# zfw1226/active_tracking_rl

Measured on AMD Instinct MI355X. Metric: env steps/sec, Track2D-BlockPartialPZR-v0 @4096 envs, 1/2/4/8 GPU, higher is better.
Workload: dtype u8 map bits / f64 reward -> f32 obs+reward; policy fp32

## Files before the change

### active_tracking_rl_amd/build.py

```python
import os
import re
import subprocess
import sys
from concurrent.futures import ThreadPoolExecutor

HERE = os.path.dirname(os.path.abspath(__file__))
CSRC = os.path.join(HERE, "csrc")
OBJ = os.path.join(CSRC, "_obj")
LIB = os.path.join(HERE, "libtrack2d_hip.so")
SOURCES = ["track2d_hip.hip", "stem_hip.hip", "policy_hip.hip", "lstm_hip.hip", "heads_hip.hip", "gemm_tn_hip.hip",
           "actor_step_hip.hip", "pair_gemm_hip.hip", "bptt_hip.hip", "driver_hip.hip", "gate_cell_hip.hip", "episode_stats_hip.hip",
           "gru_hip.hip", "np_mode.cpp", "lt_gemm.cpp"]
HEADERS = ["t2d_device.h", os.path.join("..", "..", "include", "track2d.h"),
           os.path.join("..", "..", "include", "atr_policy.h"), "atr_sample.h", "atr_cell.h",
           os.path.join("..", "..", "include", "track2d_np.h"), os.path.join("..", "..", "include", "atr_eval.h"),
           os.path.join("..", "..", "include", "atr_stats.h"), os.path.join("..", "..", "include", "atr_gru.h"),
           os.path.join("..", "..", "include", "atr_gru_step.h"), os.path.join("..", "..", "include", "atr_gru_sums.h")]
HIPCC = os.environ.get("HIPCC", "/opt/rocm/bin/hipcc")
CFLAGS = ["--offload-arch=gfx950", "-O3", "-std=c++17", "-ffp-contract=off", "-fPIC", "-Wno-unused-result"]
LDFLAGS = ["--offload-arch=gfx950", "-fPIC", "-shared", "-ldl"]
NO_SCRATCH = {"track2d_hip.hip": "k_gru_step"}
NO_SCRATCH_LEARNER = {"gru_hip.hip": "k_gru_bptt"}
REMARKS = "-Rpass-analysis=kernel-resource-usage"


def _newest_header():
    return max(os.path.getmtime(os.path.join(CSRC, h)) for h in HEADERS)


def _obj(src):
    return os.path.join(OBJ, os.path.splitext(src)[0] + ".o")


def _stale(src, hdr_time):
    o = _obj(src)
    return not os.path.exists(o) or os.path.getmtime(o) < max(os.path.getmtime(os.path.join(CSRC, src)), hdr_time)


def needs_build():
    if not os.path.exists(LIB):
        return True
    t = os.path.getmtime(LIB)
    return any(os.path.getmtime(os.path.join(CSRC, f)) > t for f in SOURCES + HEADERS)


# ... 4 lines not shown
        if m:
            name = m.group(1)
            seen += part in name
            continue
        m = re.search(r"remark:\s+ScratchSize \[bytes/lane\]: (\d+)", line)
        if m and name is not None and part in name and int(m.group(1)) != 0:
            bad.append((name, int(m.group(1))))
    if not seen:
        raise RuntimeError("no resource remark names a %s kernel: the scratch check found nothing to check" % part)
    return bad


def build(force=False, verbose=False):
    if not force and not needs_build():
        return LIB
    os.makedirs(OBJ, exist_ok=True)
    hdr_time = _newest_header()
    todo = [s for s in SOURCES if force or _stale(s, hdr_time)]

    def compile_one(src):
        cmd = [HIPCC] + CFLAGS + ["-c", os.path.join(CSRC, src), "-o", _obj(src)]
        if verbose:
            print(" ".join(cmd), flush=True)
        part = NO_SCRATCH.get(src) or NO_SCRATCH_LEARNER.get(src)
        if part is None:
            subprocess.check_call(cmd)
            return
        r = subprocess.run(cmd + [REMARKS], stderr=subprocess.PIPE, text=True)
        if r.returncode != 0:
            sys.stderr.write(r.stderr)
            raise subprocess.CalledProcessError(r.returncode, cmd)
        sys.stderr.write("".join(l + "\n" for l in r.stderr.splitlines() if "warning:" in l))
        bad = scratch_users(r.stderr, part)
        if bad:
            os.remove(_obj(src))
            raise RuntimeError("%s: scratch memory in %s" % (src, ", ".join("%s (%d bytes per lane)" % b for b in bad)))
    with ThreadPoolExecutor(max_workers=min(len(todo), os.cpu_count() or 4) or 1) as pool:
        list(pool.map(compile_one, todo))
    cmd = [HIPCC] + LDFLAGS + ["-o", LIB] + [_obj(s) for s in SOURCES]
    if verbose:
        print(" ".join(cmd), flush=True)
    subprocess.check_call(cmd)
    return LIB


if __name__ == "__main__":
    print(build(force="--force" in sys.argv, verbose=True))
# ... 1 lines not shown
```

### active_tracking_rl_amd/csrc/heads_hip.hip

```cpp
#include <hip/hip_runtime.h>
#include <stdint.h>

#include "../../include/atr_policy.h"

namespace atr {

constexpr int kHeadsMaxA = 8;
constexpr int kHeadsBlock = 256;

__device__ __forceinline__ float4 h_ld4(const float *p) { return *reinterpret_cast<const float4 *>(p); }
__device__ __forceinline__ float dot4(const float4 &a, const float4 &b) { return fmaf(a.x, b.x, fmaf(a.y, b.y, fmaf(a.z, b.z, a.w * b.w))); }
__device__ __forceinline__ float row_sum(float v, int L)
{
    v += __builtin_bit_cast(float, __builtin_amdgcn_update_dpp(0, __builtin_bit_cast(int, v), 0xB1 , 0xf, 0xf, true));
    v += __builtin_bit_cast(float, __builtin_amdgcn_update_dpp(0, __builtin_bit_cast(int, v), 0x4E , 0xf, 0xf, true));
    v += __builtin_bit_cast(float, __builtin_amdgcn_update_dpp(0, __builtin_bit_cast(int, v), 0x124 , 0xf, 0xf, true));
    v += __builtin_bit_cast(float, __builtin_amdgcn_update_dpp(0, __builtin_bit_cast(int, v), 0x128 , 0xf, 0xf, true));
    if (L > 16) v += __shfl_xor(v, 16, 64);
    if (L > 32) v += __shfl_xor(v, 32, 64);
    return v;
}

__global__ __launch_bounds__(kHeadsBlock) void k_heads_values(const float *__restrict__ h, const float *__restrict__ wc,
                                                              const float *__restrict__ bc, float *__restrict__ values,
                                                              long long rows, int R, int vstride, int voff,
                                                              const float *__restrict__ h1, const float *__restrict__ wc1,
                                                              const float *__restrict__ bc1, int voff1)
{
    const int half = h1 ? (int)(gridDim.x >> 1) : (int)gridDim.x;
    const bool second = h1 && (int)blockIdx.x >= half;
    if (second) { h = h1; wc = wc1; bc = bc1; voff = voff1; }
    const int bid = second ? (int)blockIdx.x - half : (int)blockIdx.x;
    const int L = R >> 2;
    const long long total = rows * L;
// ... 46 lines not shown
    const float4 wc = h_ld4(a.wc + j);
    const float4 wx = a.waux ? h_ld4(a.waux + j) : make_float4(0.f, 0.f, 0.f, 0.f);
    const long long rstride = (long long)nblk * slots;
    long long row = (long long)bid * slots + slot;
    float4 hv_n = make_float4(0.f, 0.f, 0.f, 0.f);
    float v_n = 0.f, ret_n = 0.f, gae_n = 0.f, raux_n = 0.f;
    int act_n_ = 0;
    auto fetch = [&](long long r) {
        if (r < a.rows) {
            hv_n = h_ld4(a.h + r * a.R + j);
            const long long s_ = r * a.stride + a.off;
            v_n = a.val[s_]; ret_n = a.ret[s_]; gae_n = a.gae[s_];
            const unsigned an_ = (unsigned)(a.act_n > 0x7fffffffLL ? 0x7fffffffLL : a.act_n), at_ = (unsigned)r / an_;
            act_n_ = (int)a.actions[(long long)at_ * a.act_tstride + (long long)((unsigned)r - at_ * an_)];
            if (a.r_aux) raux_n = a.r_aux[r * a.aux_stride + a.aux_off];
        }
    };
    fetch(row);
    for (; row < a.rows; row += rstride) {
        const float4 hv = hv_n;
        const float v = v_n, ret = ret_n, gae = gae_n, raux = raux_n;
        const int act = act_n_;
        fetch(row + rstride);
        float z[NAx];
#pragma unroll
        for (int i = 0; i < NAx; i++) z[i] = i < A ? row_sum(dot4(hv, wa[i]), L) + a.ba[i] : -INFINITY;
        const float pred = a.waux ? row_sum(dot4(hv, wx), L) + a.baux[0] : 0.f;
        float mx = z[0];
#pragma unroll
        for (int i = 1; i < NAx; i++) mx = fmaxf(mx, z[i]);
        float p[NAx], se = 0.f;
#pragma unroll
        for (int i = 0; i < NAx; i++) { p[i] = i < A ? expf(z[i] - mx) : 0.f; se += p[i]; }
        const float lse = mx + logf(se);
        float ent = 0.f, logp_a = 0.f;
#pragma unroll
        for (int i = 0; i < NAx; i++) {
            if (i < A) {
                p[i] = p[i] / se;
                const float lp = z[i] - lse;
                ent -= lp * p[i];
                if (i == act) logp_a = lp;
            }
        }
        const float dlogp = -a.scale * gae, dent = -a.scale * a.w_ent;
        const float dv = a.scale * 0.5f * (v - ret);
        float dpred = 0.f, aux_abs = 0.f;
        if (a.r_aux) {
            const float diff = pred - raux;
            aux_abs = fabsf(diff);
            dpred = a.scale_aux * (diff > 0.f ? 1.f : (diff < 0.f ? -1.f : 0.f));
        }
        float dz[NAx];
#pragma unroll
        for (int i = 0; i < NAx; i++)
            dz[i] = i < A ? dlogp * ((i == act ? 1.f : 0.f) - p[i]) - dent * p[i] * ((z[i] - lse) + ent) : 0.f;
        float4 dh = make_float4(dv * wc.x + dpred * wx.x, dv * wc.y + dpred * wx.y, dv * wc.z + dpred * wx.z, dv * wc.w + dpred * wx.w);
#pragma unroll
        for (int i = 0; i < NAx; i++)
            if (i < A) {
                dh.x = fmaf(dz[i], wa[i].x, dh.x); dh.y = fmaf(dz[i], wa[i].y, dh.y);
                dh.z = fmaf(dz[i], wa[i].z, dh.z); dh.w = fmaf(dz[i], wa[i].w, dh.w);
                gwa[i].x = fmaf(dz[i], hv.x, gwa[i].x); gwa[i].y = fmaf(dz[i], hv.y, gwa[i].y);
                gwa[i].z = fmaf(dz[i], hv.z, gwa[i].z); gwa[i].w = fmaf(dz[i], hv.w, gwa[i].w);
                gba[i] += dz[i];
            }
        {
            float *dp = a.dh + row * a.R + j;
            __builtin_nontemporal_store(dh.x, dp); __builtin_nontemporal_store(dh.y, dp + 1);
            __builtin_nontemporal_store(dh.z, dp + 2); __builtin_nontemporal_store(dh.w, dp + 3);
        }
        gwc.x = fmaf(dv, hv.x, gwc.x); gwc.y = fmaf(dv, hv.y, gwc.y); gwc.z = fmaf(dv, hv.z, gwc.z); gwc.w = fmaf(dv, hv.w, gwc.w);
        gwx.x = fmaf(dpred, hv.x, gwx.x); gwx.y = fmaf(dpred, hv.y, gwx.y); gwx.z = fmaf(dpred, hv.z, gwx.z); gwx.w = fmaf(dpred, hv.w, gwx.w);
        gbc += dv; gbx += dpred;
        s_pol += -logp_a * gae - a.w_ent * ent;
        s_val += 0.5f * (ret - v) * (ret - v);
        s_ent += ent;
        s_aux += aux_abs;
    }
    __shared__ float4 wred[kHeadsBlock];
    const int rec = (A + 2) * a.R + (A + 2) + 4;
    float *out = a.partial + (size_t)bid * rec;
#pragma unroll
    for (int q = 0; q < NAx + 2; q++) {
        if (q < A + 2) {
            float4 g = gwx;
            if (q < NAx && q < A) g = gwa[q < NAx ? q : 0];
            else if (q == A) g = gwc;
            __syncthreads();
            wred[threadIdx.x] = g;
            __syncthreads();
            if (slot == 0) {
                float4 acc = wred[threadIdx.x];
                for (int sl = 1; sl < slots; sl++) {
                    const float4 t = wred[sl * L + (int)threadIdx.x];
                    acc.x += t.x; acc.y += t.y; acc.z += t.z; acc.w += t.w;
                }
                *reinterpret_cast<float4 *>(out + q * a.R + j) = acc;
            }
        }
    }
    __syncthreads();
    if (j == 0) {
#pragma unroll
        for (int i = 0; i < NAx; i++) red[slot][i] = gba[i];
        red[slot][kHeadsMaxA] = gbc; red[slot][kHeadsMaxA + 1] = gbx;
        red[slot][kHeadsMaxA + 2] = s_pol; red[slot][kHeadsMaxA + 3] = s_val;
        red[slot][kHeadsMaxA + 4] = s_ent; red[slot][kHeadsMaxA + 5] = s_aux;
    }
    __syncthreads();
    if (threadIdx.x < (unsigned)(A + 2 + 4)) {
        const int q = (int)threadIdx.x;
        const int src = q < A ? q : kHeadsMaxA + (q - A);
        float acc = 0.f;
        for (int sl = 0; sl < slots; sl++) acc += red[sl][src];
        out[(A + 2) * a.R + q] = acc;
    }
}

struct HeadsReduce {
    const float *partial[2];
    float *out[2];
    float *stats_out[2];
    float scale[2], scale_aux[2];
    int nrec[2];
    float stats_scale;
    int rec, nb, fold;
};

__global__ __launch_bounds__(1024) void k_heads_reduce(const HeadsReduce f)
{
    __shared__ float red[64][17];
    __shared__ float tail[16];
    const int pi = (int)blockIdx.x >= f.nb ? 1 : 0, b = (int)blockIdx.x - pi * f.nb;
    const float *__restrict__ partial = f.partial[pi];
    float *__restrict__ out = f.out[pi];
    const int nrec = f.nrec[pi], rec = f.rec;
    const int jl = (int)(threadIdx.x & 15u), slice = (int)(threadIdx.x >> 4);
    const int j = b * 16 + jl;
    float acc = 0.f;
// ... 86 lines not shown
    for (int i = 0; i < 2; i++) {
        const atr_heads_loss_args &p = players[i < count ? i : 0];
        if (heads_fill(g.p[i], p) != 0) return -1;
        if (i >= count) g.p[i].grid = 0;
        f.partial[i] = p.workspace; f.out[i] = p.grads_and_sums; f.stats_out[i] = p.stats_out; f.scale[i] = p.scale;
        f.scale_aux[i] = p.scale_aux; f.nrec[i] = g.p[i].grid;
    }
    if (count == 2 && (players[0].R != players[1].R || players[0].A != players[1].A)) return -1;
    const int rec = (players[0].A + 2) * players[0].R + (players[0].A + 2) + 4;
    f.stats_scale = stats_scale; f.rec = rec; f.nb = (rec + 15) / 16; f.fold = (rec - 4) / 16 == (rec - 1) / 16 ? 1 : 0;
    hipStream_t st = (hipStream_t)stream;
    if (players[0].A <= 4)
        hipLaunchKernelGGL(k_heads_loss<4>, dim3((unsigned)(g.p[0].grid + g.p[1].grid)), dim3(kHeadsBlock), 0, st, g);
    else
        hipLaunchKernelGGL(k_heads_loss<kHeadsMaxA>, dim3((unsigned)(g.p[0].grid + g.p[1].grid)), dim3(kHeadsBlock), 0, st, g);
    hipLaunchKernelGGL(k_heads_reduce, dim3((unsigned)(f.nb * count)), dim3(1024), 0, st, f);
    if (!f.fold)
        for (int i = 0; i < count; i++)
            hipLaunchKernelGGL(k_heads_finish, dim3(1), dim3(1), 0, st, players[i].grads_and_sums, rec, players[i].scale,
                               players[i].scale_aux, players[i].stats_out, stats_scale);
    return hipGetLastError() == hipSuccess ? 0 : -2;
}

extern "C" int atr_heads_loss(const float *h, const long long *actions, const float *ret, const float *gae,
                              const float *val, int stride, int off, const float *r_aux, int aux_stride, int aux_off,
                              const float *wa, const float *ba, const float *wc, const float *waux, const float *baux,
                              float scale, float scale_aux, float w_ent, float *dh, float *grads_and_sums,
                              float *workspace, long long rows, int R, int A, void *stream)
{
    atr_heads_loss_args p = {};
    p.h = h; p.actions = actions; p.act_n = rows > 0 ? rows : 1; p.act_tstride = 0; p.ret = ret; p.gae = gae; p.val = val;
    p.stride = stride; p.off = off; p.r_aux = r_aux; p.aux_stride = aux_stride; p.aux_off = aux_off; p.wa = wa; p.ba = ba;
    p.wc = wc; p.waux = waux; p.baux = baux; p.scale = scale; p.scale_aux = scale_aux; p.w_ent = w_ent; p.dh = dh;
    p.grads_and_sums = grads_and_sums; p.workspace = workspace; p.stats_out = nullptr; p.rows = rows; p.R = R; p.A = A;
    return atr_heads_loss_multi(&p, 1, 1.0f, stream);
}
```

### active_tracking_rl_amd/fused.py

```python
import ctypes as C
import json
import os
import re
import sys

import torch

from . import vec_env

_lib = None


class ActStepArgs(C.Structure):
    _fields_ = [("ig", C.c_void_p * 2), ("hg", C.c_void_p * 2), ("bias", C.c_void_p * 2), ("c_prev", C.c_void_p * 2),
                ("h_out", C.c_void_p * 2), ("c_out", C.c_void_p * 2), ("acts", C.c_void_p * 2),
                ("actor_w", C.c_void_p * 2), ("actor_b", C.c_void_p * 2), ("emb", C.c_void_p), ("done_prev", C.c_void_p),
                ("actions_out", C.c_void_p), ("counter", C.c_void_p), ("seed", C.c_ulonglong), ("ordinal", C.c_uint),
                ("A", C.c_int), ("N", C.c_int), ("R", C.c_int), ("hm_out", C.c_void_p * 2), ("hm_ld", C.c_longlong)]


class CoopStepArgs(C.Structure):
    _fields_ = [("y", C.c_void_p * 2), ("fc_w", C.c_void_p * 2), ("fc_b", C.c_void_p * 2), ("w_cat", C.c_void_p * 2),
                ("ldy", C.c_longlong * 2), ("kfc", C.c_int * 2), ("fh", C.c_void_p), ("gates", C.c_void_p),
                ("fh_pstride", C.c_longlong), ("fh_ld", C.c_longlong), ("F", C.c_int), ("workgroups", C.c_int),
# ... 119 lines not shown


ATR_PROTOTYPES = _prototypes()
GRU_PROTOTYPES = {
    "atr_gru_cell_forward": (C.c_int, [C.c_void_p] * 6 + [C.c_longlong, C.c_void_p, C.c_void_p, C.c_void_p, C.c_longlong,
                                       C.c_void_p, C.c_longlong, C.c_int, C.c_int, C.c_int, C.c_void_p]),
    "atr_gru_cell_backward": (C.c_int, [C.c_void_p, C.c_longlong, C.c_void_p, C.c_void_p, C.c_void_p, C.c_void_p, C.c_longlong,
                                        C.c_void_p, C.c_longlong, C.c_void_p, C.c_longlong, C.c_int, C.c_int, C.c_int, C.c_int,
                                        C.c_void_p]),
    "atr_gru_bptt": (C.c_int, [C.c_void_p] * 4 + [C.c_longlong, C.c_void_p, C.c_longlong, C.c_void_p, C.c_void_p, C.c_void_p,
                               C.c_longlong, C.c_void_p, C.c_int, C.c_int, C.c_int, C.c_int, C.c_void_p]),
}
GRU_SUMS_PROTOTYPES = {
    "atr_gru_bptt_act_sums_floats": (C.c_longlong, [C.c_int]),
    "atr_gru_bptt_sums": (C.c_int, GRU_PROTOTYPES["atr_gru_bptt"][1][:12] + [C.c_int, C.c_int, C.c_void_p, C.c_longlong, C.c_void_p,
                                                                            C.c_int, C.c_int, C.c_int, C.c_int, C.c_void_p]),
}
GRU_STEP_PROTOTYPES = {
    "atr_gru_act_env_step": (C.c_int, [C.c_void_p, C.POINTER(ActStepArgs), C.c_void_p, C.c_void_p, C.c_longlong, C.c_void_p,
                                       C.c_int, C.c_void_p, C.c_void_p, C.c_void_p]),
    "atr_gru_eval_act_env_step": (C.c_int, [C.c_void_p, C.POINTER(ActStepArgs), C.c_void_p, C.c_void_p, C.c_longlong, C.c_void_p,
                                            C.c_void_p, C.c_int, C.c_void_p, C.c_void_p, C.c_void_p]),
}
_ERROR_DETAIL = {"atr_act_env_step": "t2d_last_error", "atr_coop_env_step": "t2d_last_error", "atr_linear": "atr_lt_last_error"}
_GRU_STEP_ERROR_DETAIL = {name: "t2d_last_error" for name in GRU_STEP_PROTOTYPES}


def _errcheck(name):
    def check(status, func=None, args=None):
        if status != 0:
            text = _ERROR_DETAIL.get(name) or _GRU_STEP_ERROR_DETAIL.get(name)
            detail = ": " + getattr(lib(), text)().decode() if text else ""
            raise RuntimeError("%s failed (%d)%s" % (name, status, detail))
        return status
    return check


def lib():
    global _lib
    if _lib is None:
        L = vec_env.load_library()
        for name, (restype, argtypes, *value) in (list(ATR_PROTOTYPES.items()) + list(GRU_PROTOTYPES.items())
                                                  + list(GRU_SUMS_PROTOTYPES.items()) + list(GRU_STEP_PROTOTYPES.items())):
            f = getattr(L, name)
            f.restype, f.argtypes = restype, argtypes
            if restype is C.c_int and not value:
                f.errcheck = _errcheck(name)
        _lib = L
    return _lib


def _p(t):
    return C.c_void_p(t.data_ptr())


def _stem_fn(name, x):
    if x.dtype == torch.uint8:
        return getattr(lib(), name + "_u8")
    if x.dtype != torch.float32:
        raise TypeError("stem frames must be float32 or uint8, got %s" % x.dtype)
    return getattr(lib(), name)


def _stream(t):
    return C.c_void_p(torch.cuda.current_stream(t.device).cuda_stream)

# ... 1130 lines not shown
        return hs[0][1][hs[0][5]], hs[1][1][hs[1][5]], stats

    @staticmethod
    def backward(ctx, g0, g1, gstats):
        sv = ctx.saved_tensors
        out = [None]
        for p in range(2):
            if (g0, g1)[p] is None:
                out += [None] * 7
            else:
                out += _head_grads(sv[2 * p], sv[2 * p + 1], *ctx.dims[p])
        return tuple(out)


def heads_loss_pair(hs, actors, critics, auxes, cfg):
    t = []
    for p in range(2):
        aux = auxes[p]
        t += [hs[p], actors[p].weight, actors[p].bias, critics[p].weight, critics[p].bias,
              aux.weight if aux is not None else None, aux.bias if aux is not None else None]
    return _HeadsLossPair.apply(cfg, *t)


class _HeadsLoss(torch.autograd.Function):

    @staticmethod
    def forward(ctx, h, wa, ba, wc, bc, waux, baux, actions, ret, gae, val, off, r_aux, aux_off, scale, scale_aux, w_ent,
                unit_coeff=False):
        L = lib()
        h = h.contiguous()
        rows, R = h.shape
        A = wa.shape[0]
        stride = _col_stride(ret)
        rec = (A + 2) * R + (A + 2) + 4
        dh = torch.empty_like(h)
        gs = torch.empty(rec + 1, dtype=torch.float32, device=h.device)
        ws = torch.empty(L.atr_heads_workspace_floats(rows, R, A), dtype=torch.float32, device=h.device)
        actions = actions.contiguous()
        aux_stride = _col_stride(r_aux) if r_aux is not None else 0
        L.atr_heads_loss(_p(h), _p(actions), _p(ret), _p(gae), _p(val), stride, off, _pn(r_aux), aux_stride, aux_off,
                         _p(wa), _p(ba), _p(wc), _pn(waux), _pn(baux), float(scale), float(scale_aux), float(w_ent),
                         _p(dh), _p(gs), _p(ws), rows, R, A, _stream(h))
        ctx.save_for_backward(dh, gs)
        ctx.dims = (A, R, waux is not None)
        ctx.unit_coeff = bool(unit_coeff)
        stats = gs[rec - 4:rec]
# ... 270 lines not shown
```

### active_tracking_rl_amd/player_util.py

```python
import torch
import torch.distributed as dist


class Agent(object):
    def __init__(self, model, env, args, state, device):
        self.model = model
        self.env = env
        self.num_agents = len(env.observation_space)
        self.num_envs = getattr(env, "num_envs", 1)
        if 'continuous' in args.network:
            raise NotImplementedError("continuous actions belong to the Unreal envs (out of scope)")
        self.dim_action = 1
        self.args = args
        self.device = device
        self.rnn_out = args.rnn_out
        self.values, self.log_probs, self.rewards, self.entropies, self.preds, self.dones = [], [], [], [], [], []
        self.states, self.actions, self.h0, self.c0 = [], [], None, None
        self._buf, self._pending_done, self._cache, self._actions_buf = None, None, None, None
        self.cache_rollout = True
        self.fused_heads = True
        self.fused_bookkeeping = True
        self._keep = None
        self.carry_out, self.carry_written, self._want_loss_terms = None, (), False
        self.greedy_eval = None
# ... 319 lines not shown
        pred_loss = (preds - rewards[:, :, 0]).abs().sum(0) if use_aux else torch.zeros(N, 1, device=dev)
        loss_tracker = (policy_loss[:, 0] + 0.5 * value_loss[:, 0]).mean()
        loss_target = (policy_loss[:, 1] + 0.5 * value_loss[:, 1]).mean() if A > 1 else 0
        if training_mode == 0:
            loss = loss_tracker
        elif training_mode == 1:
            loss = loss_target
        else:
            loss = loss_tracker + loss_target
        if use_aux and training_mode != 0:
            loss = loss + pred_loss.mean()
        return loss, policy_loss, value_loss, entropies.detach().sum(0), pred_loss

    def _loss_fused_heads(self, training_mode, states, actions, rewards, nd):
        from . import fused
        args, model = self.args, self.model
        T, N, A = self._cache.T, self.num_envs, self.num_agents
        dev = self.device
        players = (model.player0, model.player1)
        need = (training_mode != 1, training_mode != 0) if A == 2 else None
        h_seq = model.cached_hidden(self._cache, states, actions, nd, need)
        R_dim = h_seq[0].shape[-1]
        v = torch.empty((T + 1, N, A, 1), dtype=torch.float32, device=dev)
        with torch.no_grad():
            if A == 2:
                fused.heads_values2([h_seq[p].detach().reshape(T * N, R_dim) for p in range(2)],
                                    [players[p].critic.critic_linear for p in range(2)], v)
            else:
                for p in range(A):
                    fused.heads_values(h_seq[p].detach().reshape(T * N, R_dim), players[p].critic.critic_linear, v, p)
            sampler = getattr(model, "_sampler", None)
            if hasattr(model, "boot_values") and sampler is not None and getattr(sampler, "_last", None) is not None:
                sampler.reopen_block()
                model.boot_values(self.state, self._cache, self.done, v[T])
                sampler.end_block()
            else:
                k_end = (self.done == 0).to(torch.float32).view(N, 1, 1)
                hx_end = self._cache.h_all[:, T].transpose(0, 1) * k_end
                cx_end = self._cache.c_all[:, T].transpose(0, 1) * k_end
                boot, _, _, _, _, _ = model((self.state, (hx_end, cx_end)))
                v[T].copy_(boot)
            R, gae = fused.gae_returns(rewards.contiguous(), v, nd, args.gamma, args.tau)
        use_aux = 'reward' in args.aux and getattr(model, "tat", False) and getattr(model.player1, "sub_task", False)
        w_ent = [float(args.entropy)] + [float(self.w_entropy_target)] * (A - 1)
        scale = [1.0 / N if training_mode in (0, -1) else 0.0, 1.0 / N if training_mode in (1, -1) else 0.0]
        if training_mode not in (0, 1, -1):
            scale = [1.0 / N, 1.0 / N]
        scale_aux = 1.0 / N if (use_aux and training_mode != 0) else 0.0
        rew_c = rewards.contiguous()
        if A == 2 and players[0].actor.actor_linear.weight.shape == players[1].actor.actor_linear.weight.shape:
            cfg = []
            for p in range(2):
                aux = players[p].reward_aux if (p == 1 and use_aux) else None
                cfg.append(dict(actions=actions[:, :, p], ret=R, gae=gae, val=v, off=p, r_aux=rew_c if aux is not None else None,
                                aux_off=0, scale=scale[p], scale_aux=scale_aux if aux is not None else 0.0, w_ent=w_ent[p],
                                stats_scale=1.0 / N))
            auxes = [None, players[1].reward_aux if use_aux else None]
            l0, l1, st = fused.heads_loss_pair([h_seq[p].reshape(T * N, R_dim) for p in range(2)],
                                               [players[p].actor.actor_linear for p in range(2)],
                                               [players[p].critic.critic_linear for p in range(2)], auxes, cfg)
            loss = (l0, l1) if getattr(self, "_want_loss_terms", False) else l0 + l1
        else:
            loss, stats = 0, []
            for p in range(A):
                aux = players[p].reward_aux if (p == 1 and use_aux) else None
                lp, st_ = fused.heads_loss(h_seq[p].reshape(T * N, R_dim), players[p].actor.actor_linear,
                                           players[p].critic.critic_linear, aux, actions[:, :, p].reshape(T * N), R, gae, v, p,
                                           rew_c if aux is not None else None, 0, scale[p], scale_aux if aux is not None else 0.0,
                                           w_ent[p], unit_coeff=True)
                loss = loss + lp
                stats.append(st_)
            st = torch.stack(stats, 0) / N
        policy_loss, value_loss, entropies = (st[:, k].reshape(1, A, 1) for k in range(3))
        pred_loss = st[1, 3].reshape(1, 1) if (A > 1 and use_aux) else torch.zeros(1, 1, device=dev)
        return loss, policy_loss, value_loss, entropies, pred_loss

    def compute_grads(self, optimizer, training_mode):
        fast = len(self.states) > 0
        bucket = getattr(optimizer, "bucket", None)
        self._want_loss_terms = bucket is not None and hasattr(bucket, "set_grads")
        try:
            loss, policy_loss, value_loss, entropies, pred_loss = (self.loss_recompute if fast else self.loss)(training_mode)
        finally:
# ... 57 lines not shown
```

### include/atr_policy.h

```cpp
#ifndef ATR_POLICY_H
#define ATR_POLICY_H

#ifdef __cplusplus
extern "C" {
#endif

int atr_stem_forward(const float *x, long long x_stride, const float *w1, const float *b1, const float *w2,
                     const float *b2, float *y, long long M, void *stream);
int atr_stem_forward2(const float *x0, long long x0_stride, const float *w1_0, const float *b1_0, const float *w2_0,
                      const float *b2_0, float *y0, long long M0, const float *x1, long long x1_stride,
                      const float *w1_1, const float *b1_1, const float *w2_1, const float *b2_1, float *y1,
                      long long M1, void *stream);
long long atr_stem_workspace_floats(long long M);
int atr_stem_backward(const float *x, long long x_stride, const float *y, const float *dy, const float *w1,
                      const float *b1, const float *w2, float *dw1, float *db1, float *dw2, float *db2,
                      float *workspace, long long M, void *stream);

int atr_stem_forward_u8(const unsigned char *x, long long x_stride, const float *w1, const float *b1, const float *w2,
                        const float *b2, float *y, long long M, void *stream);
int atr_stem_forward2_u8(const unsigned char *x0, long long x0_stride, const float *w1_0, const float *b1_0,
                         const float *w2_0, const float *b2_0, float *y0, long long M0, const unsigned char *x1,
                         long long x1_stride, const float *w1_1, const float *b1_1, const float *w2_1,
                         const float *b2_1, float *y1, long long M1, void *stream);
int atr_stem_backward_u8(const unsigned char *x, long long x_stride, const float *y, const float *dy, const float *w1,
// ... 155 lines not shown
int atr_heads_values2(const float *h, const float *wc, const float *bc, int voff, const float *h1, const float *wc1,
                      const float *bc1, int voff1, float *values, long long rows, int R, int vstride, void *stream);
long long atr_heads_workspace_floats(long long rows, int R, int A);
int atr_heads_loss(const float *h, const long long *actions, const float *ret, const float *gae, const float *val,
                   int stride, int off, const float *r_aux, int aux_stride, int aux_off, const float *wa,
                   const float *ba, const float *wc, const float *waux, const float *baux, float scale, float scale_aux,
                   float w_ent, float *dh, float *grads_and_sums, float *workspace, long long rows, int R, int A,
                   void *stream);
typedef struct atr_heads_loss_args {
    const float *h;
    const long long *actions;
    long long act_n, act_tstride;
    const float *ret, *gae, *val;
    int stride, off;
    const float *r_aux;
    int aux_stride, aux_off;
    const float *wa, *ba, *wc, *waux, *baux;
    float scale, scale_aux, w_ent;
    float *dh, *grads_and_sums, *workspace, *stats_out;
    long long rows;
    int R, A;
} atr_heads_loss_args;
int atr_heads_loss_multi(const atr_heads_loss_args *players, int count, float stats_scale, void *stream);

long long atr_gemm_tn_workspace_floats(long long K, int M, int N);
int atr_gemm_tn(const float *x1, const float *x2, float *c, float *workspace, long long K, int M, int N,
                const float *row_scale, float *colsum, void *stream);

#define atr_scatter_max_segments 64
int atr_scatter_segments(const float *const *src, const long long *dst_off, const int *n, int count, float *dst, void *stream);

typedef struct atr_gemm_tn_problem {
    const float *x1, *x2;
    float *c;
    const float *row_scale;
    long long row_scale_shift;
    float *colsum0, *colsum1;
    int M, N;
    long long ld1, ld2;
} atr_gemm_tn_problem;
long long atr_gemm_tn_grouped_workspace_floats(const atr_gemm_tn_problem *problems, int count, long long K);
int atr_gemm_tn_set_corun(int on);
int atr_gemm_tn_grouped(const atr_gemm_tn_problem *problems, int count, long long K, float *workspace, void *stream);

int atr_rollout_begin(const float *hxs, const float *cxs, float *h0, float *c0, long long pstride, const void *obs_src,
                      void *obs_dst, long long obs_bytes, int N, int A, int R, void *stream);
typedef struct atr_rollout_consts {
    const float *w_ih[2], *w_hh[2], *b_ih[2], *b_hh[2];
    float *bsum, *w_cat;
    const float *fa_w, *fa_b;
    float *emb_ih;
    unsigned long long *counter;
    float *fh0;
    long long fh_pstride, fh_ld;
    int F, A_act;
} atr_rollout_consts;
int atr_rollout_begin2(const float *hxs, const float *cxs, float *h0, float *c0, long long pstride, const void *obs_src,
                       void *obs_dst, long long obs_bytes, int N, int A, int R, const atr_rollout_consts *consts, void *stream);
int atr_rollout_end(const float *hT, const float *cT, long long pstride, const uint8_t *dones, float *hxs, float *cxs,
                    int *eps_len, float *keep, int T, int N, int A, int R, void *stream);
int atr_rollout_end2(const float *hT, const float *cT, long long pstride, const uint8_t *dones, float *hxs, float *cxs,
                     int *eps_len, float *keep, int T, int N, int A, int R, const void *obs_src, void *obs_dst,
                     long long obs_bytes, uint8_t *done_dst, void *stream);
int atr_adam_step(float *params, const float *grad, float *exp_avg, float *exp_avg_sq, float *max_exp_avg_sq, double *state,
                  float *scalars, double lr, double beta1, double beta2, double eps, double weight_decay, int torch_eps,
                  long long n, void *stream);
int atr_rmsprop_step(float *params, const float *grad, float *square_avg, double lr, double alpha, double eps,
                     double weight_decay, long long n, void *stream);

#ifdef __cplusplus
}
#endif
#endif
```

Baseline: 17.48 million.

## Fuse critic values, GAE returns and head loss into one front kernel

Adds a k_heads_front kernel that computes critic values for each timestep, runs the GAE/returns backward scan within a 32-lane group per env, and then evaluates the actor/critic/aux head loss and gradients, all in one pass. The separate heads_values2 and gae_returns launches are skipped when shapes match (2 agents, R=128, A=4, T<=32). The intent is to remove kernel launches and the round trips of values, returns and advantages through global memory. In exchange, h is read twice, each env is processed serially by a 32-lane slot, and the fast path only covers a narrow set of shapes.

```diff
diff --git a/active_tracking_rl_amd/build.py b/active_tracking_rl_amd/build.py
--- a/active_tracking_rl_amd/build.py
+++ b/active_tracking_rl_amd/build.py
@@ -15,12 +15,14 @@
            os.path.join("..", "..", "include", "atr_policy.h"), "atr_sample.h", "atr_cell.h",
            os.path.join("..", "..", "include", "track2d_np.h"), os.path.join("..", "..", "include", "atr_eval.h"),
            os.path.join("..", "..", "include", "atr_stats.h"), os.path.join("..", "..", "include", "atr_gru.h"),
-           os.path.join("..", "..", "include", "atr_gru_step.h"), os.path.join("..", "..", "include", "atr_gru_sums.h")]
+           os.path.join("..", "..", "include", "atr_gru_step.h"), os.path.join("..", "..", "include", "atr_gru_sums.h"),
+           os.path.join("..", "..", "include", "atr_heads_front.h"), "heads_row.inc", "heads_block_reduce.inc"]
 HIPCC = os.environ.get("HIPCC", "/opt/rocm/bin/hipcc")
 CFLAGS = ["--offload-arch=gfx950", "-O3", "-std=c++17", "-ffp-contract=off", "-fPIC", "-Wno-unused-result"]
 LDFLAGS = ["--offload-arch=gfx950", "-fPIC", "-shared", "-ldl"]
 NO_SCRATCH = {"track2d_hip.hip": "k_gru_step"}
 NO_SCRATCH_LEARNER = {"gru_hip.hip": "k_gru_bptt"}
+NO_SCRATCH_HEADS = {"heads_hip.hip": "k_heads_front"}
 REMARKS = "-Rpass-analysis=kernel-resource-usage"
 
 
@@ -71,7 +73,7 @@
         cmd = [HIPCC] + CFLAGS + ["-c", os.path.join(CSRC, src), "-o", _obj(src)]
         if verbose:
             print(" ".join(cmd), flush=True)
-        part = NO_SCRATCH.get(src) or NO_SCRATCH_LEARNER.get(src)
+        part = NO_SCRATCH.get(src) or NO_SCRATCH_LEARNER.get(src) or NO_SCRATCH_HEADS.get(src)
         if part is None:
             subprocess.check_call(cmd)
             return
diff --git a/active_tracking_rl_amd/csrc/heads_block_reduce.inc b/active_tracking_rl_amd/csrc/heads_block_reduce.inc
--- /dev/null
+++ b/active_tracking_rl_amd/csrc/heads_block_reduce.inc
@@ -0,0 +1,38 @@
+    __shared__ float4 wred[kHeadsBlock];
+    const int rec = (A + 2) * a.R + (A + 2) + 4;
+    float *out = a.partial + (size_t)bid * rec;
+#pragma unroll
+    for (int q = 0; q < NAx + 2; q++) {
+        if (q < A + 2) {
+            float4 g = gwx;
+            if (q < NAx && q < A) g = gwa[q < NAx ? q : 0];
+            else if (q == A) g = gwc;
+            __syncthreads();
+            wred[threadIdx.x] = g;
+            __syncthreads();
+            if (slot == 0) {
+                float4 acc = wred[threadIdx.x];
+                for (int sl = 1; sl < slots; sl++) {
+                    const float4 t = wred[sl * L + (int)threadIdx.x];
+                    acc.x += t.x; acc.y += t.y; acc.z += t.z; acc.w += t.w;
+                }
+                *reinterpret_cast<float4 *>(out + q * a.R + j) = acc;
+            }
+        }
+    }
+    __syncthreads();
+    if (j == 0) {
+#pragma unroll
+        for (int i = 0; i < NAx; i++) red[slot][i] = gba[i];
+        red[slot][kHeadsMaxA] = gbc; red[slot][kHeadsMaxA + 1] = gbx;
+        red[slot][kHeadsMaxA + 2] = s_pol; red[slot][kHeadsMaxA + 3] = s_val;
+        red[slot][kHeadsMaxA + 4] = s_ent; red[slot][kHeadsMaxA + 5] = s_aux;
+    }
+    __syncthreads();
+    if (threadIdx.x < (unsigned)(A + 2 + 4)) {
+        const int q = (int)threadIdx.x;
+        const int src = q < A ? q : kHeadsMaxA + (q - A);
+        float acc = 0.f;
+        for (int sl = 0; sl < slots; sl++) acc += red[sl][src];
+        out[(A + 2) * a.R + q] = acc;
+    }
diff --git a/active_tracking_rl_amd/csrc/heads_hip.hip b/active_tracking_rl_amd/csrc/heads_hip.hip
--- a/active_tracking_rl_amd/csrc/heads_hip.hip
+++ b/active_tracking_rl_amd/csrc/heads_hip.hip
@@ -10,6 +10,10 @@
 
 __device__ __forceinline__ float4 h_ld4(const float *p) { return *reinterpret_cast<const float4 *>(p); }
 __device__ __forceinline__ float dot4(const float4 &a, const float4 &b) { return fmaf(a.x, b.x, fmaf(a.y, b.y, fmaf(a.z, b.z, a.w * b.w))); }
+__device__ __forceinline__ float h_uniform(float v)
+{
+    return __builtin_bit_cast(float, __builtin_amdgcn_readfirstlane(__builtin_bit_cast(int, v)));
+}
 __device__ __forceinline__ float row_sum(float v, int L)
 {
     v += __builtin_bit_cast(float, __builtin_amdgcn_update_dpp(0, __builtin_bit_cast(int, v), 0xB1 , 0xf, 0xf, true));
@@ -102,100 +106,100 @@
         const float v = v_n, ret = ret_n, gae = gae_n, raux = raux_n;
         const int act = act_n_;
         fetch(row + rstride);
-        float z[NAx];
-#pragma unroll
-        for (int i = 0; i < NAx; i++) z[i] = i < A ? row_sum(dot4(hv, wa[i]), L) + a.ba[i] : -INFINITY;
-        const float pred = a.waux ? row_sum(dot4(hv, wx), L) + a.baux[0] : 0.f;
-        float mx = z[0];
-#pragma unroll
-        for (int i = 1; i < NAx; i++) mx = fmaxf(mx, z[i]);
-        float p[NAx], se = 0.f;
-#pragma unroll
-        for (int i = 0; i < NAx; i++) { p[i] = i < A ? expf(z[i] - mx) : 0.f; se += p[i]; }
-        const float lse = mx + logf(se);
-        float ent = 0.f, logp_a = 0.f;
-#pragma unroll
-        for (int i = 0; i < NAx; i++) {
-            if (i < A) {
-                p[i] = p[i] / se;
-                const float lp = z[i] - lse;
-                ent -= lp * p[i];
-                if (i == act) logp_a = lp;
+#include "heads_row.inc"
+    }
+#include "heads_block_reduce.inc"
+}
+
+constexpr int kFrontLoads = 5;
+struct HeadsFront {
+    HeadsLoss p[2];
+    const float *bc[2];
+    const float *rew, *nd;
+    float *values;
+    float *ret_out, *gae_out;
+    float gamma, tau;
+    int T, N;
+};
+
+template <int NAx>
+__global__ __launch_bounds__(kHeadsBlock) __attribute__((amdgpu_waves_per_eu(4))) void k_heads_front(const HeadsFront g)
+{
+    const int pi = (int)blockIdx.x >= g.p[0].grid ? 1 : 0;
+    HeadsLoss a = g.p[pi];
+    float ba_r[kHeadsMaxA], baux_r = a.baux ? h_uniform(a.baux[0]) : 0.f;
+#pragma unroll
+    for (int i = 0; i < kHeadsMaxA; i++) ba_r[i] = i < NAx ? h_uniform(a.ba[i]) : 0.f;
+    a.ba = ba_r; a.baux = &baux_r;
+    a.R = 128;
+    const int bid = (int)blockIdx.x - (pi ? g.p[0].grid : 0), nblk = a.grid;
+    __shared__ float red[kHeadsBlock / 16][(kHeadsMaxA + 2) * 4 + 1];
+    constexpr int L = 32, R = 128, slots = kHeadsBlock / L;
+    constexpr int A = NAx;
+    const int T = g.T, N = g.N;
+    const int slot = (int)threadIdx.x / L, l = (int)threadIdx.x % L;
+    const int j = l * 4;
+    float4 gwa[NAx], gwc = make_float4(0.f, 0.f, 0.f, 0.f), gwx = gwc;
+    float gba[NAx], gbc = 0.f, gbx = 0.f, s_pol = 0.f, s_val = 0.f, s_ent = 0.f, s_aux = 0.f;
+#pragma unroll
+    for (int i = 0; i < NAx; i++) { gwa[i] = make_float4(0.f, 0.f, 0.f, 0.f); gba[i] = 0.f; }
+    float4 wa[NAx];
+#pragma unroll
+    for (int i = 0; i < NAx; i++) wa[i] = h_ld4(a.wa + i * R + j);
+    const float4 wc = h_ld4(a.wc + j);
+    const float4 wx = a.waux ? h_ld4(a.waux + j) : make_float4(0.f, 0.f, 0.f, 0.f);
+    const float bc = h_uniform(g.bc[pi][0]);
+    const long long tstep = (long long)N * R;
+    for (int n = bid * slots + slot; n < N; n += nblk * slots) {
+        const unsigned jn = (unsigned)n * R + j;
+        const float boot = g.values[((long long)T * N + n) * a.stride + a.off];
+        float rew_l = 0.f, nd_l = 0.f, raux_l = 0.f;
+        int act_l = 0;
+        const long long r_l = (long long)l * N + n, s_l = r_l * a.stride + a.off;
+        if (l < T) {
+            rew_l = g.rew[s_l]; nd_l = g.nd[r_l];
+            const unsigned an_ = (unsigned)(a.act_n > 0x7fffffffLL ? 0x7fffffffLL : a.act_n), at_ = (unsigned)r_l / an_;
+            act_l = (int)a.actions[(long long)at_ * a.act_tstride + (long long)((unsigned)r_l - at_ * an_)];
+            if (a.r_aux) raux_l = a.r_aux[r_l * a.aux_stride + a.aux_off];
+        }
+        float v_l = 0.f;
+        for (int t0 = 0; t0 < T; t0 += kFrontLoads) {
+            float4 x[kFrontLoads];
+#pragma unroll
+            for (int u = 0; u < kFrontLoads; u++) x[u] = h_ld4(a.h + (t0 + u < T ? t0 + u : T - 1) * tstep + jn);
+#pragma unroll
+            for (int u = 0; u < kFrontLoads; u++) {
+                const float vt = row_sum(dot4(x[u], wc), L) + bc;
+                if (l == t0 + u && t0 + u < T) v_l = vt;
             }
         }
-        const float dlogp = -a.scale * gae, dent = -a.scale * a.w_ent;
-        const float dv = a.scale * 0.5f * (v - ret);
-        float dpred = 0.f, aux_abs = 0.f;
-        if (a.r_aux) {
-            const float diff = pred - raux;
-            aux_abs = fabsf(diff);
-            dpred = a.scale_aux * (diff > 0.f ? 1.f : (diff < 0.f ? -1.f : 0.f));
-        }
-        float dz[NAx];
-#pragma unroll
-        for (int i = 0; i < NAx; i++)
-            dz[i] = i < A ? dlogp * ((i == act ? 1.f : 0.f) - p[i]) - dent * p[i] * ((z[i] - lse) + ent) : 0.f;
-        float4 dh = make_float4(dv * wc.x + dpred * wx.x, dv * wc.y + dpred * wx.y, dv * wc.z + dpred * wx.z, dv * wc.w + dpred * wx.w);
-#pragma unroll
-        for (int i = 0; i < NAx; i++)
-            if (i < A) {
-                dh.x = fmaf(dz[i], wa[i].x, dh.x); dh.y = fmaf(dz[i], wa[i].y, dh.y);
-                dh.z = fmaf(dz[i], wa[i].z, dh.z); dh.w = fmaf(dz[i], wa[i].w, dh.w);
-                gwa[i].x = fmaf(dz[i], hv.x, gwa[i].x); gwa[i].y = fmaf(dz[i], hv.y, gwa[i].y);
-                gwa[i].z = fmaf(dz[i], hv.z, gwa[i].z); gwa[i].w = fmaf(dz[i], hv.w, gwa[i].w);
-                gba[i] += dz[i];
-            }
-        {
-            float *dp = a.dh + row * a.R + j;
-            __builtin_nontemporal_store(dh.x, dp); __builtin_nontemporal_store(dh.y, dp + 1);
-            __builtin_nontemporal_store(dh.z, dp + 2); __builtin_nontemporal_store(dh.w, dp + 3);
-        }
-        gwc.x = fmaf(dv, hv.x, gwc.x); gwc.y = fmaf(dv, hv.y, gwc.y); gwc.z = fmaf(dv, hv.z, gwc.z); gwc.w = fmaf(dv, hv.w, gwc.w);
-        gwx.x = fmaf(dpred, hv.x, gwx.x); gwx.y = fmaf(dpred, hv.y, gwx.y); gwx.z = fmaf(dpred, hv.z, gwx.z); gwx.w = fmaf(dpred, hv.w, gwx.w);
-        gbc += dv; gbx += dpred;
-        s_pol += -logp_a * gae - a.w_ent * ent;
-        s_val += 0.5f * (ret - v) * (ret - v);
-        s_ent += ent;
-        s_aux += aux_abs;
-    }
-    __shared__ float4 wred[kHeadsBlock];
-    const int rec = (A + 2) * a.R + (A + 2) + 4;
-    float *out = a.partial + (size_t)bid * rec;
-#pragma unroll
-    for (int q = 0; q < NAx + 2; q++) {
-        if (q < A + 2) {
-            float4 g = gwx;
-            if (q < NAx && q < A) g = gwa[q < NAx ? q : 0];
-            else if (q == A) g = gwc;
-            __syncthreads();
-            wred[threadIdx.x] = g;
-            __syncthreads();
-            if (slot == 0) {
-                float4 acc = wred[threadIdx.x];
-                for (int sl = 1; sl < slots; sl++) {
-                    const float4 t = wred[sl * L + (int)threadIdx.x];
-                    acc.x += t.x; acc.y += t.y; acc.z += t.z; acc.w += t.w;
-                }
-                *reinterpret_cast<float4 *>(out + q * a.R + j) = acc;
-            }
-        }
-    }
-    __syncthreads();
-    if (j == 0) {
-#pragma unroll
-        for (int i = 0; i < NAx; i++) red[slot][i] = gba[i];
-        red[slot][kHeadsMaxA] = gbc; red[slot][kHeadsMaxA + 1] = gbx;
-        red[slot][kHeadsMaxA + 2] = s_pol; red[slot][kHeadsMaxA + 3] = s_val;
-        red[slot][kHeadsMaxA + 4] = s_ent; red[slot][kHeadsMaxA + 5] = s_aux;
-    }
-    __syncthreads();
-    if (threadIdx.x < (unsigned)(A + 2 + 4)) {
-        const int q = (int)threadIdx.x;
-        const int src = q < A ? q : kHeadsMaxA + (q - A);
-        float acc = 0.f;
-        for (int sl = 0; sl < slots; sl++) acc += red[sl][src];
-        out[(A + 2) * a.R + q] = acc;
-    }
+        if (l < T) g.values[s_l] = v_l;
+        const float vup = __shfl_down(v_l, 1, L);
+        const float v1 = l == T - 1 ? boot : vup;
+        const float delta_l = rew_l + g.gamma * v1 * nd_l - v_l;
+        float r_run = boot, g_run = 0.0f, ret_l = 0.f, gae_l = 0.f;
+        for (int t = T - 1; t >= 0; t--) {
+            const float k = __shfl(nd_l, t, L), r = __shfl(rew_l, t, L), delta = __shfl(delta_l, t, L);
+            r_run = g.gamma * r_run * k + r;
+            g_run = g_run * g.gamma * g.tau * k + delta;
+            if (l == t) { ret_l = r_run; gae_l = g_run; }
+        }
+        if (l < T) {
+            if (g.ret_out) g.ret_out[s_l] = ret_l;
+            if (g.gae_out) g.gae_out[s_l] = gae_l;
+        }
+        float4 hv_n = h_ld4(a.h + jn);
+        for (int t = 0; t < T; t++) {
+            const float4 hv = hv_n;
+            if (t + 1 < T) hv_n = h_ld4(a.h + (t + 1) * tstep + jn);
+            const float v = __shfl(v_l, t, L), ret = __shfl(ret_l, t, L), gae = __shfl(gae_l, t, L), raux = __shfl(raux_l, t, L);
+            const int act = __shfl(act_l, t, L);
+            const long long row = (long long)t * N;
+            const unsigned j = jn;
+#include "heads_row.inc"
+        }
+    }
+#include "heads_block_reduce.inc"
 }
 
 struct HeadsReduce {
@@ -328,6 +332,48 @@
     return hipGetLastError() == hipSuccess ? 0 : -2;
 }
 
+static int heads_front_grid(int N)
+{
+    const int b = (N + 7) / 8;
+    return b > 512 ? 512 : (b < 1 ? 1 : b);
+}
+
+extern "C" long long atr_heads_front_workspace_floats(int N, int R, int A)
+{
+    if (N < 1 || R != 128 || A != 4) return -1;
+    return (long long)heads_front_grid(N) * ((A + 2) * R + (A + 2) + 4);
+}
+
+extern "C" int atr_heads_front(const atr_heads_loss_args *players, int count, const float *bc0, const float *bc1,
+                               const float *rewards, const float *notdone, float *values, float gamma, float tau, int T, int N,
+                               float *ret, float *gae, float stats_scale, void *stream)
+{
+    if (!players || count != 2 || !bc0 || !bc1 || !rewards || !notdone || !values || T < 1 || T > 32 || N < 1 || N > (1 << 23)) return -1;
+    HeadsFront g;
+    HeadsReduce f;
+    for (int i = 0; i < 2; i++) {
+        atr_heads_loss_args p = players[i];
+        if (p.R != 128 || p.A != 4 || p.stride != players[0].stride || p.rows != (long long)T * N) return -1;
+        p.ret = p.gae = p.val = values;
+        if (heads_fill(g.p[i], p) != 0) return -1;
+        g.p[i].grid = heads_front_grid(N);
+        f.partial[i] = p.workspace; f.out[i] = p.grads_and_sums; f.stats_out[i] = p.stats_out; f.scale[i] = p.scale;
+        f.scale_aux[i] = p.scale_aux; f.nrec[i] = g.p[i].grid;
+    }
+    g.bc[0] = bc0; g.bc[1] = bc1; g.rew = rewards; g.nd = notdone; g.values = values; g.ret_out = ret; g.gae_out = gae;
+    g.gamma = gamma; g.tau = tau; g.T = T; g.N = N;
+    const int rec = (players[0].A + 2) * 128 + (players[0].A + 2) + 4;
+    f.stats_scale = stats_scale; f.rec = rec; f.nb = (rec + 15) / 16; f.fold = (rec - 4) / 16 == (rec - 1) / 16 ? 1 : 0;
+    hipStream_t st = (hipStream_t)stream;
+    hipLaunchKernelGGL(k_heads_front<4>, dim3((unsigned)(g.p[0].grid + g.p[1].grid)), dim3(kHeadsBlock), 0, st, g);
+    hipLaunchKernelGGL(k_heads_reduce, dim3((unsigned)(f.nb * 2)), dim3(1024), 0, st, f);
+    if (!f.fold)
+        for (int i = 0; i < 2; i++)
+            hipLaunchKernelGGL(k_heads_finish, dim3(1), dim3(1), 0, st, players[i].grads_and_sums, rec, players[i].scale,
+                               players[i].scale_aux, players[i].stats_out, stats_scale);
+    return hipGetLastError() == hipSuccess ? 0 : -2;
+}
+
 extern "C" int atr_heads_loss(const float *h, const long long *actions, const float *ret, const float *gae,
                               const float *val, int stride, int off, const float *r_aux, int aux_stride, int aux_off,
                               const float *wa, const float *ba, const float *wc, const float *waux, const float *baux,
diff --git a/active_tracking_rl_amd/csrc/heads_row.inc b/active_tracking_rl_amd/csrc/heads_row.inc
--- /dev/null
+++ b/active_tracking_rl_amd/csrc/heads_row.inc
@@ -0,0 +1,55 @@
+        float z[NAx];
+#pragma unroll
+        for (int i = 0; i < NAx; i++) z[i] = i < A ? row_sum(dot4(hv, wa[i]), L) + a.ba[i] : -INFINITY;
+        const float pred = a.waux ? row_sum(dot4(hv, wx), L) + a.baux[0] : 0.f;
+        float mx = z[0];
+#pragma unroll
+        for (int i = 1; i < NAx; i++) mx = fmaxf(mx, z[i]);
+        float p[NAx], se = 0.f;
+#pragma unroll
+        for (int i = 0; i < NAx; i++) { p[i] = i < A ? expf(z[i] - mx) : 0.f; se += p[i]; }
+        const float lse = mx + logf(se);
+        float ent = 0.f, logp_a = 0.f;
+#pragma unroll
+        for (int i = 0; i < NAx; i++) {
+            if (i < A) {
+                p[i] = p[i] / se;
+                const float lp = z[i] - lse;
+                ent -= lp * p[i];
+                if (i == act) logp_a = lp;
+            }
+        }
+        const float dlogp = -a.scale * gae, dent = -a.scale * a.w_ent;
+        const float dv = a.scale * 0.5f * (v - ret);
+        float dpred = 0.f, aux_abs = 0.f;
+        if (a.r_aux) {
+            const float diff = pred - raux;
+            aux_abs = fabsf(diff);
+            dpred = a.scale_aux * (diff > 0.f ? 1.f : (diff < 0.f ? -1.f : 0.f));
+        }
+        float dz[NAx];
+#pragma unroll
+        for (int i = 0; i < NAx; i++)
+            dz[i] = i < A ? dlogp * ((i == act ? 1.f : 0.f) - p[i]) - dent * p[i] * ((z[i] - lse) + ent) : 0.f;
+        float4 dh = make_float4(dv * wc.x + dpred * wx.x, dv * wc.y + dpred * wx.y, dv * wc.z + dpred * wx.z, dv * wc.w + dpred * wx.w);
+#pragma unroll
+        for (int i = 0; i < NAx; i++)
+            if (i < A) {
+                dh.x = fmaf(dz[i], wa[i].x, dh.x); dh.y = fmaf(dz[i], wa[i].y, dh.y);
+                dh.z = fmaf(dz[i], wa[i].z, dh.z); dh.w = fmaf(dz[i], wa[i].w, dh.w);
+                gwa[i].x = fmaf(dz[i], hv.x, gwa[i].x); gwa[i].y = fmaf(dz[i], hv.y, gwa[i].y);
+                gwa[i].z = fmaf(dz[i], hv.z, gwa[i].z); gwa[i].w = fmaf(dz[i], hv.w, gwa[i].w);
+                gba[i] += dz[i];
+            }
+        {
+            float *dp = a.dh + row * a.R + j;
+            __builtin_nontemporal_store(dh.x, dp); __builtin_nontemporal_store(dh.y, dp + 1);
+            __builtin_nontemporal_store(dh.z, dp + 2); __builtin_nontemporal_store(dh.w, dp + 3);
+        }
+        gwc.x = fmaf(dv, hv.x, gwc.x); gwc.y = fmaf(dv, hv.y, gwc.y); gwc.z = fmaf(dv, hv.z, gwc.z); gwc.w = fmaf(dv, hv.w, gwc.w);
+        gwx.x = fmaf(dpred, hv.x, gwx.x); gwx.y = fmaf(dpred, hv.y, gwx.y); gwx.z = fmaf(dpred, hv.z, gwx.z); gwx.w = fmaf(dpred, hv.w, gwx.w);
+        gbc += dv; gbx += dpred;
+        s_pol += -logp_a * gae - a.w_ent * ent;
+        s_val += 0.5f * (ret - v) * (ret - v);
+        s_ent += ent;
+        s_aux += aux_abs;
diff --git a/active_tracking_rl_amd/fused.py b/active_tracking_rl_amd/fused.py
--- a/active_tracking_rl_amd/fused.py
+++ b/active_tracking_rl_amd/fused.py
@@ -165,6 +165,12 @@
     "atr_gru_eval_act_env_step": (C.c_int, [C.c_void_p, C.POINTER(ActStepArgs), C.c_void_p, C.c_void_p, C.c_longlong, C.c_void_p,
                                             C.c_void_p, C.c_int, C.c_void_p, C.c_void_p, C.c_void_p]),
 }
+HEADS_FRONT_PROTOTYPES = {
+    "atr_heads_front_workspace_floats": (C.c_longlong, [C.c_int, C.c_int, C.c_int]),
+    "atr_heads_front": (C.c_int, [C.POINTER(HeadsLossArgs), C.c_int] + [C.c_void_p] * 5 + [C.c_float, C.c_float, C.c_int, C.c_int,
+                                                                                          C.c_void_p, C.c_void_p, C.c_float,
+                                                                                          C.c_void_p], VALUE),
+}
 _ERROR_DETAIL = {"atr_act_env_step": "t2d_last_error", "atr_coop_env_step": "t2d_last_error", "atr_linear": "atr_lt_last_error"}
 _GRU_STEP_ERROR_DETAIL = {name: "t2d_last_error" for name in GRU_STEP_PROTOTYPES}
 
@@ -184,7 +190,8 @@
     if _lib is None:
         L = vec_env.load_library()
         for name, (restype, argtypes, *value) in (list(ATR_PROTOTYPES.items()) + list(GRU_PROTOTYPES.items())
-                                                  + list(GRU_SUMS_PROTOTYPES.items()) + list(GRU_STEP_PROTOTYPES.items())):
+                                                  + list(GRU_SUMS_PROTOTYPES.items()) + list(GRU_STEP_PROTOTYPES.items())
+                                                  + list(HEADS_FRONT_PROTOTYPES.items())):
             f = getattr(L, name)
             f.restype, f.argtypes = restype, argtypes
             if restype is C.c_int and not value:
@@ -1361,6 +1368,86 @@
     return _HeadsLossPair.apply(cfg, *t)
 
 
+heads_front = os.environ.get("ATR_HEADS_FRONT", "1") != "0"
+
+
+def heads_front_ok(T, agents, R, actor_shapes, h_contiguous, enabled=None):
+    enabled = heads_front if enabled is None else enabled
+    shapes = [tuple(x) for x in actor_shapes]
+    return bool(enabled and agents == 2 and len(shapes) == 2 and 1 <= T <= 32 and R == 128 and shapes[0] == shapes[1] == (4, R)
+                and len(h_contiguous) == 2 and all(h_contiguous))
+
+
+class _HeadsFrontPair(torch.autograd.Function):
+
+    @staticmethod
+    def forward(ctx, cfg, shared, *t):
+        L = lib()
+        rewards, notdone, values, gamma, tau, ret, gae = shared
+        arr = (HeadsLossArgs * 2)()
+        hs, keep = [], []
+        for p in range(2):
+            h, wa, ba, wc, bc, waux, baux = t[7 * p:7 * p + 7]
+            c = cfg[p]
+            T, N, R = h.shape
+            A = wa.shape[0]
+            rec = (A + 2) * R + (A + 2) + 4
+            dh = torch.empty_like(h)
+            gs = torch.empty(rec + 1, dtype=torch.float32, device=h.device)
+            ws = torch.empty(max(L.atr_heads_front_workspace_floats(N, R, A), 1), dtype=torch.float32, device=h.device)
+            acts, act_n, act_ts = _act_layout(c["actions"], T * N)
+            a = arr[p]
+            a.h, a.actions, a.act_n, a.act_tstride = h.data_ptr(), acts.data_ptr(), act_n, act_ts
+            a.stride = _col_stride(values)
+            a.off = c["off"]
+            r_aux = c.get("r_aux")
+            a.r_aux = r_aux.data_ptr() if r_aux is not None else None
+            a.aux_stride = _col_stride(r_aux) if r_aux is not None else 0
+            a.aux_off = c.get("aux_off", 0)
+            a.wa, a.ba, a.wc = wa.data_ptr(), ba.data_ptr(), wc.data_ptr()
+            a.waux = waux.data_ptr() if waux is not None else None
+            a.baux = baux.data_ptr() if baux is not None else None
+            a.scale, a.scale_aux, a.w_ent = float(c["scale"]), float(c["scale_aux"]), float(c["w_ent"])
+            a.dh, a.grads_and_sums, a.workspace = dh.data_ptr(), gs.data_ptr(), ws.data_ptr()
+            a.rows, a.R, a.A = T * N, R, A
+            hs.append((dh, gs, A, R, waux is not None, rec, bc))
+            keep += [h, acts, ws]
+        T, N = t[0].shape[0], t[0].shape[1]
+        stats = torch.empty((2, 4), dtype=torch.float32, device=hs[0][0].device)
+        arr[0].stats_out, arr[1].stats_out = stats.data_ptr(), stats.data_ptr() + 16
+        status = L.atr_heads_front(arr, 2, _p(hs[0][6]), _p(hs[1][6]), _p(rewards), _p(notdone), _p(values), float(gamma),
+                                   float(tau), T, N, _pn(ret), _pn(gae), float(cfg[0]["stats_scale"]), _stream(hs[0][0]))
+        if status != 0:
+            raise RuntimeError("atr_heads_front: status %d (heads_front_ok() names the shapes it has a kernel for)" % status)
+        ctx.save_for_backward(hs[0][0], hs[0][1], hs[1][0], hs[1][1])
+        ctx.dims = [(x[2], x[3], x[4]) for x in hs]
+        ctx.set_materialize_grads(False)
+        ctx.mark_non_differentiable(stats)
+        return hs[0][1][hs[0][5]], hs[1][1][hs[1][5]], stats
+
+    @staticmethod
+    def backward(ctx, g0, g1, gstats):
+        sv = ctx.saved_tensors
+        out = [None, None]
+        for p in range(2):
+            if (g0, g1)[p] is None:
+                out += [None] * 7
+            else:
+                out += _head_grads(sv[2 * p], sv[2 * p + 1], *ctx.dims[p])
+        return tuple(out)
+
+
+def heads_front_pair(hs, actors, critics, auxes, cfg, rewards, notdone, values, gamma, tau, ret=None, gae=None):
+    assert rewards.is_contiguous() and notdone.is_contiguous() and values.is_contiguous()
+    assert all(h.dim() == 3 and h.is_contiguous() for h in hs) and hs[0].shape == hs[1].shape
+    t = []
+    for p in range(2):
+        aux = auxes[p]
+        t += [hs[p], actors[p].weight, actors[p].bias, critics[p].weight, critics[p].bias,
+              aux.weight if aux is not None else None, aux.bias if aux is not None else None]
+    return _HeadsFrontPair.apply(cfg, (rewards, notdone, values, gamma, tau, ret, gae), *t)
+
+
 class _HeadsLoss(torch.autograd.Function):
 
     @staticmethod
diff --git a/active_tracking_rl_amd/player_util.py b/active_tracking_rl_amd/player_util.py
--- a/active_tracking_rl_amd/player_util.py
+++ b/active_tracking_rl_amd/player_util.py
@@ -365,8 +365,12 @@
         h_seq = model.cached_hidden(self._cache, states, actions, nd, need)
         R_dim = h_seq[0].shape[-1]
         v = torch.empty((T + 1, N, A, 1), dtype=torch.float32, device=dev)
+        front = fused.heads_front_ok(T, A, R_dim, [players[p].actor.actor_linear.weight.shape for p in range(A)],
+                                     [h.dim() == 3 and h.is_contiguous() for h in h_seq])
         with torch.no_grad():
-            if A == 2:
+            if front:
+                pass
+            elif A == 2:
                 fused.heads_values2([h_seq[p].detach().reshape(T * N, R_dim) for p in range(2)],
                                     [players[p].critic.critic_linear for p in range(2)], v)
             else:
@@ -383,7 +387,7 @@
                 cx_end = self._cache.c_all[:, T].transpose(0, 1) * k_end
                 boot, _, _, _, _, _ = model((self.state, (hx_end, cx_end)))
                 v[T].copy_(boot)
-            R, gae = fused.gae_returns(rewards.contiguous(), v, nd, args.gamma, args.tau)
+            R, gae = (None, None) if front else fused.gae_returns(rewards.contiguous(), v, nd, args.gamma, args.tau)
         use_aux = 'reward' in args.aux and getattr(model, "tat", False) and getattr(model.player1, "sub_task", False)
         w_ent = [float(args.entropy)] + [float(self.w_entropy_target)] * (A - 1)
         scale = [1.0 / N if training_mode in (0, -1) else 0.0, 1.0 / N if training_mode in (1, -1) else 0.0]
@@ -399,9 +403,14 @@
                                 aux_off=0, scale=scale[p], scale_aux=scale_aux if aux is not None else 0.0, w_ent=w_ent[p],
                                 stats_scale=1.0 / N))
             auxes = [None, players[1].reward_aux if use_aux else None]
-            l0, l1, st = fused.heads_loss_pair([h_seq[p].reshape(T * N, R_dim) for p in range(2)],
-                                               [players[p].actor.actor_linear for p in range(2)],
-                                               [players[p].critic.critic_linear for p in range(2)], auxes, cfg)
+            if front:
+                l0, l1, st = fused.heads_front_pair(h_seq, [players[p].actor.actor_linear for p in range(2)],
+                                                    [players[p].critic.critic_linear for p in range(2)], auxes, cfg, rew_c,
+                                                    nd.contiguous(), v, args.gamma, args.tau)
+            else:
+                l0, l1, st = fused.heads_loss_pair([h_seq[p].reshape(T * N, R_dim) for p in range(2)],
+                                                   [players[p].actor.actor_linear for p in range(2)],
+                                                   [players[p].critic.critic_linear for p in range(2)], auxes, cfg)
             loss = (l0, l1) if getattr(self, "_want_loss_terms", False) else l0 + l1
         else:
             loss, stats = 0, []
diff --git a/include/atr_heads_front.h b/include/atr_heads_front.h
--- /dev/null
+++ b/include/atr_heads_front.h
@@ -0,0 +1,17 @@
+#ifndef ATR_HEADS_FRONT_H
+#define ATR_HEADS_FRONT_H
+
+#ifdef __cplusplus
+extern "C" {
+#endif
+
+long long atr_heads_front_workspace_floats(int N, int R, int A);
+int atr_heads_front(const atr_heads_loss_args *players, int count, const float *bc0, const float *bc1, const float *rewards,
+                    const float *notdone, float *values, float gamma, float tau, int T, int N, float *ret, float *gae,
+                    float stats_scale, void *stream);
+
+#ifdef __cplusplus
+}
+#endif
+
+#endif
diff --git a/include/atr_policy.h b/include/atr_policy.h
--- a/include/atr_policy.h
+++ b/include/atr_policy.h
@@ -201,7 +201,6 @@
     int R, A;
 } atr_heads_loss_args;
 int atr_heads_loss_multi(const atr_heads_loss_args *players, int count, float stats_scale, void *stream);
-
 long long atr_gemm_tn_workspace_floats(long long K, int M, int N);
 int atr_gemm_tn(const float *x1, const float *x2, float *c, float *workspace, long long K, int M, int N,
                 const float *row_scale, float *colsum, void *stream);
@@ -247,6 +246,8 @@
 int atr_rmsprop_step(float *params, const float *grad, float *square_avg, double lr, double alpha, double eps,
                      double weight_decay, long long n, void *stream);
 
+#include "atr_heads_front.h"
+
 #ifdef __cplusplus
 }
 #endif
```

New measurement: 17.48 million, median of 2. Within noise of the previous version (-0.0%).
